# Jorgenlf/Drone-2d-custom-gym-env-for-reinforcement-learning

Measured on AMD Instinct MI355X. Metric: env-steps/sec at 65 536 parallel envs; 1/2/4/8 MI355X scaling, higher is better.
Workload: dtype f64

## Files before the change

### drone-2d-custom-gym-env-for-reinforcement-learning_amd/csrc/d2d_device.h

```cpp
#pragma once
#include <hip/hip_runtime.h>
#include <stdint.h>

#include "../../include/drone2d.h"
#include "d2d_pmath.h"

#pragma clang diagnostic ignored "-Wbitwise-instead-of-logical"

#ifdef D2D_BSTAMP
#define BST_N (1024 * 64 * 8)
__device__ uint64_t d2d_bst[BST_N];
#define BST_ARG , uint64_t* bst = nullptr
#define BST(k, dep)                                                                                      \
    do {                                                                                                 \
        if (bst) {                                                                                       \
            uint64_t bst_v;                                                                              \
            asm volatile("s_memtime %0\n\ts_waitcnt lgkmcnt(0)" : "=s"(bst_v) : "v"(dep));            \
            bst_t[k] = bst_v;                                                                            \
        }                                                                                                \
    } while (0)
#else
#define BST_ARG
#define BST(k, dep) \
    do {       \
// ... 564 lines not shown
        const double t = le ? xf : x;
        const int ti = le ? B.ixf : ix;
        const double tk = le ? B.kxf : kx;
        B.a = to_a ? t : a;
        B.b = to_a ? b : t;
        B.ia = to_a ? ti : B.ia;
        B.ka = to_a ? tk : B.ka;
        B.ib = to_a ? B.ib : ti;
        B.ixf = le ? ix : B.ixf;
        B.kxf = le ? kx : B.kxf;
        const int j = k + 1;
        const double nfulc = (le | c1) ? nfc : fulc;
        const int njf = (le | c1) ? jn : jf;
        const double nnfc = le ? xf : (c1 ? x : nfc);
        const int njn = le ? jx : (c1 ? j : jn);
        B.fulc = nfulc;
        B.nfc = nnfc;
        B.xf = le ? x : xf;
        jf = njf;
        jn = njn;
        jx = le ? j : jx;
    }
    T.snap[kind][k] = BtSnap{B.a, B.b, B.fulc, B.nfc, B.xf, B.rat, B.e, B.ka, B.kxf, B.num, B.ia, B.ib, B.ixf,
                             jf, jn, jx, 0};
    T.len[kind] = k;
}

__device__ __forceinline__ double bt_check(const BtIt& h, int k, double px, double py, double ffulc, double fnfc,
                                           double fx, int& dev) {
    const double fu = norm2(h.X - px, h.Y - py);
    const double r = h.dxn * (fx - ffulc);
    double q = h.dxf * (fx - fnfc);
    double p = h.dxf * q - h.dxn * r;
    q = 2.0 * (q - r);
    p = (q > 0.0) ? -p : p;
    q = fabs(q);
    const bool par = (fabs(p) < fabs(0.5 * q * h.e)) & (p > q * h.am) & (p < q * h.bm);
    const bool ok = !par & (fu <= fx);
    dev = min(dev, ok ? BT_HOT : k);
    return fu;
}

template <bool LT>
__device__ __forceinline__ BtIt bt_hot(const BtHot* hot, int kind, int j) {
    if (!LT) return hot->it[kind][j];
    using HL = __attribute__((address_space(3))) const double;
    const HL* q = (const HL*)&hot->it[kind][j];
    return BtIt{q[0], q[1], q[2], q[3], q[4], q[5], q[6], q[7]};
}
template <bool LT>
__device__ __forceinline__ double bt_dist(const BtHot* hot, int kind, int j, double px, double py) {
    const BtIt h = bt_hot<LT>(hot, kind, j);
    return norm2(h.X - px, h.Y - py);
}
struct BtLane {
    int kind, len, dev;
    double fa, fb, fc;
};
template <bool LT>
__device__ __forceinline__ BtLane bt_start(const BrTab& T, const BtHot* hot, double px, double py) {
    const double f0 = bt_dist<LT>(hot, 0, 0, px, py);
    const double f1 = bt_dist<LT>(hot, 0, 1, px, py);
    BtLane L;
    L.kind = (f1 <= f0) ? 1 : 0;
    L.len = T.len[L.kind];
    L.dev = L.len;
    L.fa = f0;
    L.fb = L.kind ? f0 : f1;
    L.fc = L.kind ? f1 : f0;
    return L;
}
template <bool LT>
__device__ __forceinline__ void bt_window(const BtHot* hot, BtLane& L, int k, double px, double py) {
    L.fa = bt_dist<LT>(hot, L.kind, k - 2, px, py);
    L.fb = bt_dist<LT>(hot, L.kind, k - 1, px, py);
    L.fc = bt_dist<LT>(hot, L.kind, k, px, py);
}
template <bool LT>
__device__ __forceinline__ void bt_verify(const BtHot* hot, BtLane& L, int k0, int k1, double px, double py) {
    double fa = L.fa, fb = L.fb, fc = L.fc;
    int dev = L.dev;
    const int kind = L.kind;
    for (int k = k0; __ballot(k < min(dev, k1)) != 0ull; k += 3) {
        BtIt ha{}, hb{}, hc{};
        if (LT || k < min(dev, k1)) {
            ha = bt_hot<LT>(hot, kind, k + 1);
            hb = bt_hot<LT>(hot, kind, k + 2);
            hc = bt_hot<LT>(hot, kind, k + 3);
        }
        const double fd = bt_check(ha, k, px, py, fa, fb, fc, dev);
        const double fe = bt_check(hb, k + 1, px, py, fb, fc, fd, dev);
        const double ff = bt_check(hc, k + 2, px, py, fc, fd, fe, dev);
        fa = fd;
        fb = fe;
        fc = ff;
    }
    L.dev = min(dev, L.len);
    L.fa = fa;
    L.fb = fb;
    L.fc = fc;
}
__device__ __forceinline__ void bt_restore(const BtSnap& S, Brent& B) {
    B.a = S.a;
    B.b = S.b;
    B.fulc = S.fulc;
    B.nfc = S.nfc;
    B.xf = S.xf;
    B.rat = S.rat;
    B.e = S.e;
    B.ka = S.ka;
    B.kxf = S.kxf;
    B.num = S.num;
    B.ia = S.ia;
    B.ib = S.ib;
    B.ixf = S.ixf;
}
template <bool LT>
__device__ __forceinline__ void bt_restore_f(const BtSnap& S, const BtHot* hot, int kind, double px, double py,
                                             Brent& B) {
    B.ffulc = bt_dist<LT>(hot, kind, S.j_fulc, px, py);
    B.fnfc = bt_dist<LT>(hot, kind, S.j_nfc, px, py);
    B.fx = bt_dist<LT>(hot, kind, S.j_xf, px, py);
}
template <bool LT, class SC>
__device__ __forceinline__ double bt_finish(const SC& s, const BrTab& T, const BtHot* hot, int kind, int dev,
                                            double px, double py, int& iu) {
    const BtSnap& S = T.snap[kind][dev];
    Brent B;
    bt_restore(S, B);
    if (__ballot(brent_active(B)) != 0ull) {
        const PathK K = path_k(s);
        bt_restore_f<LT>(S, hot, kind, px, py, B);
        brent_run(s, K, px, py, B);
    }
    iu = B.ixf;
    return B.xf;
}
template <bool LT, class S>
__device__ __forceinline__ double closest_u_tab(const S& s, const BrTab& T, const BtHot* hot, double px,
                                                double py, int& iu) {
    BtLane L = bt_start<LT>(T, hot, px, py);
    bt_verify<LT>(hot, L, 1, BT_K, px, py);
    return bt_finish<LT>(s, T, hot, L.kind, L.dev, px, py, iu);
}
__device__ __forceinline__ int bt_split(const BrTab& T) { return max(4, (T.len[0] + 3) / 2); }
#ifndef D2D_BT_EARLY
#define D2D_BT_EARLY 16
#endif
constexpr int BT_EARLY = D2D_BT_EARLY;
#ifndef D2D_BT_EARLY_GRP
#define D2D_BT_EARLY_GRP 0
#endif
static_assert(BT_EARLY == 0 || (BT_EARLY >= 4 && BT_EARLY % 3 == 1 && BT_EARLY < BT_K), "BT_EARLY");
__device__ __forceinline__ int bt_third(const BrTab& T, int p) {
    const int third = (T.len[0] + 2) / 3;
    return p == 0 ? 1 : (p >= 3 ? BT_K : 1 + p * third);
}
template <bool LT>
__device__ __forceinline__ void bt_window_snap(const BrTab& T, const BtHot* hot, BtLane& L, int k0, double px,
                                               double py) {
    const BtSnap& W = T.snap[L.kind][k0];
    L.fa = bt_dist<LT>(hot, L.kind, W.j_fulc, px, py);
    L.fb = bt_dist<LT>(hot, L.kind, W.j_nfc, px, py);
    L.fc = bt_dist<LT>(hot, L.kind, W.j_xf, px, py);
}

struct Body {
    double px, py, a, vx, vy, w;
};

constexpr double M_F = 0.2, M_M = 0.4;

__host__ __device__ constexpr double moment_box(double m, double w, double h) {
    double hw = w / 2.0, hh = h / 2.0;
    double vx[4] = {hw, hw, -hw, -hw}, vy[4] = {-hh, hh, hh, -hh};
    double s1 = 0.0, s2 = 0.0;
    for (int i = 0; i < 4; ++i) {
        double v1x = vx[i] + 0.0, v1y = vy[i] + 0.0;
        double v2x = vx[(i + 1) % 4] + 0.0, v2y = vy[(i + 1) % 4] + 0.0;
        double aa = v2x * v1y - v2y * v1x;
        double bb = (v1x * v1x + v1y * v1y) + (v1x * v2x + v1y * v2y) + (v2x * v2x + v2y * v2y);
        s1 += aa * bb;
        s2 += aa;
    }
    return (m * s1) / (6.0 * s2);
}
constexpr double MI_F = 1.0 / M_F, MI_M = 1.0 / M_M;
constexpr double II_F = 1.0 / moment_box(M_F, 100.0, 10.0);
constexpr double II_M = 1.0 / moment_box(M_M, 20.0, 20.0);

struct Arms {
    double m7c[2], m7s[2];
    double f47c, f47s, f40c, f40s, f33c, f33s;
};
__device__ __forceinline__ void arm(const Arms& A, int k, double& r1x, double& r1y, double& r2x, double& r2y) {
    const int m = k < 3 ? 0 : 1;
    const int q = k % 3;
    r1x = (q == 0) ? -A.m7c[m] : ((q == 1) ? 0.0 : A.m7c[m]);
    r1y = (q == 0) ? -A.m7s[m] : ((q == 1) ? 0.0 : A.m7s[m]);
    const double c = (k == 0 || k == 5) ? A.f47c : ((k == 1 || k == 4) ? A.f40c : A.f33c);
    const double s = (k == 0 || k == 5) ? A.f47s : ((k == 1 || k == 4) ? A.f40s : A.f33s);
    r2x = (k < 3) ? -c : c;
    r2y = (k < 3) ? -s : s;
}

constexpr int ARMS_N = 10;
__device__ __forceinline__ void arms_store(const Arms& A, double* ab, int stride) {
    const double v[ARMS_N] = {A.m7c[0], A.m7c[1], A.m7s[0], A.m7s[1], A.f47c, A.f47s,
                              A.f40c, A.f40s, A.f33c, A.f33s};
#pragma unroll
    for (int q = 0; q < 10; ++q) ab[q * stride] = v[q];
}
__device__ __forceinline__ void arm_lds(const double* ab, int stride, int k, double& r1x, double& r1y, double& r2x,
                                        double& r2y) {
    using LdsD = __attribute__((address_space(3))) double;
    const volatile LdsD* v = (const volatile LdsD*)ab;
    const int m = k < 3 ? 0 : 1;
    const int q = k % 3;
    const double mc = (q == 1) ? 0.0 : v[(0 + m) * stride], ms = (q == 1) ? 0.0 : v[(2 + m) * stride];
    r1x = (q == 0) ? -mc : ((q == 1) ? 0.0 : mc);
    r1y = (q == 0) ? -ms : ((q == 1) ? 0.0 : ms);
    const int f = (k == 0 || k == 5) ? 4 : ((k == 1 || k == 4) ? 6 : 8);
    const double c = v[f * stride], sn = v[(f + 1) * stride];
    r2x = (k < 3) ? -c : c;
    r2y = (k < 3) ? -sn : sn;
}

__device__ __forceinline__ void advance_position(Body& b) {
    b.px = fma(b.vx + 0.0, DT, b.px);
    b.py = fma(b.vy + 0.0, DT, b.py);
    b.a = fma(b.w + 0.0, DT, b.a);
}
template <class S>
__device__ __forceinline__ bool frame_hits(const S& s, const Body& F, double cs, double sn) {
    bool hit = false;
    for (int k = 0; k < s.n_circles; ++k) {
        const double dx = s.cx[k] - F.px, dy = s.cy[k] - F.py;
        {
            const double reach = s.cr[k] + 51.25;
            const bool near = (fabs(dx) < reach) & (fabs(dy) < reach);
            if (__ballot(near) == 0ull) continue;
        }
        const double lx = dx * cs + dy * sn;
        const double ly = -dx * sn + dy * cs;
        const double ex = lx - fmin(fmax(lx, -FRAME_HX), FRAME_HX), ey = ly - fmin(fmax(ly, -FRAME_HY), FRAME_HY);
        const double r = s.cr[k];
        hit |= (ex * ex + ey * ey <= r * r);
    }
    return hit;
}
template <class S>
__device__ __forceinline__ bool phys_positions(const S& s, Body B[3], double fL, double fR, double cs[3],
                                               double sn[3], double& fx, double& fy, double& tq) {
    double c0, s0;
    sincos_d(B[0].a, s0, c0);
    {
        const double tx = B[0].px - (0.0 * c0 - 0.0 * s0), ty = B[0].py - (0.0 * s0 + 0.0 * c0);
        const double cgx = c0 * 0.0 + (-s0) * 0.0 + tx, cgy = s0 * 0.0 + c0 * 0.0 + ty;
        double fwx = c0 * 0.0 + (-s0) * fL, fwy = s0 * 0.0 + c0 * fL;
        double rx = (c0 * -DRONE_R + (-s0) * 0.0 + tx) - cgx, ry = (s0 * -DRONE_R + c0 * 0.0 + ty) - cgy;
        fx = 0.0 + fwx;
        fy = 0.0 + fwy;
        tq = 0.0 + (rx * fwy - ry * fwx);
        fwx = c0 * 0.0 + (-s0) * fR;
        fwy = s0 * 0.0 + c0 * fR;
        rx = (c0 * DRONE_R + (-s0) * 0.0 + tx) - cgx;
        ry = (s0 * DRONE_R + c0 * 0.0 + ty) - cgy;
        fx = fx + fwx;
        fy = fy + fwy;
        tq += rx * fwy - ry * fwx;
    }
#pragma unroll
    for (int i = 0; i < 3; ++i) advance_position(B[i]);
    sincos_d(B[0].a, sn[0], cs[0]);
#pragma unroll
    for (int i = 1; i < 3; ++i) {
        const double d = B[i].a - B[0].a;
        if (!D2D_EXACT_TRIG && fabs(d) < 1e-2) {
            const double d2 = d * d;
            const double sd = d * fma(d2, fma(d2, fma(d2, -1.0 / 5040.0, 1.0 / 120.0), -1.0 / 6.0), 1.0);
            const double cdm1 = d2 * fma(d2, fma(d2, fma(d2, 1.0 / 40320.0, -1.0 / 720.0), 1.0 / 24.0), -0.5);
            sn[i] = fma(sn[0], cdm1, fma(cs[0], sd, sn[0]));
            cs[i] = fma(cs[0], cdm1, fma(-sn[0], sd, cs[0]));
        } else {
            sincos_d(B[i].a, sn[i], cs[i]);
        }
    }
    return frame_hits(s, B[0], cs[0], sn[0]);
}
template <class S>
__device__ __forceinline__ bool frame_advance(const S& s, Body& F) {
    advance_position(F);
    double sn, cs;
    sincos_d(F.a, sn, cs);
    return frame_hits(s, F, cs, sn);
}

__device__ __forceinline__ Arms make_arms(const double cs[3], const double sn[3]) {
    Arms A;
    A.m7c[0] = cs[1] * 7.0; A.m7s[0] = sn[1] * 7.0;
    A.m7c[1] = cs[2] * 7.0; A.m7s[1] = sn[2] * 7.0;
    A.f47c = cs[0] * 47.0; A.f47s = sn[0] * 47.0;
    A.f40c = cs[0] * 40.0; A.f40s = sn[0] * 40.0;
    A.f33c = cs[0] * 33.0; A.f33s = sn[0] * 33.0;
    return A;
}
// ... 385 lines not shown
```

### drone-2d-custom-gym-env-for-reinforcement-learning_amd/csrc/d2d_kernels.h

```cpp
#pragma once
#include <type_traits>

#include "d2d_curriculum.h"
#include "d2d_device.h"
#include "d2d_layout.h"

namespace d2dk {
using namespace d2d;

constexpr int BLOCK = 256;
constexpr int K1_THREADS = 256;
constexpr size_t K1_LDS_BUDGET = 40 * 1024;
constexpr size_t K2_LDS_BUDGET = 64 * 1024;
constexpr int PRIO_W0 = 2, PRIO_W1 = 1, PRIO_W2 = 3, PRIO_W3 = 1, PRIO_W2_POST = 0;

struct StepArgs {
    int n;
    int ns;
    int n_scn;
    double* st;
    int32_t* ist;
    double* acc;
    const void* scn;
    const BrTab* brt;
// ... 45 lines not shown
            a.stamps[(size_t)(blockIdx.x * (blockDim.x >> 6) + (threadIdx.x >> 6)) * 8 + 7] =                          \
                ((uint64_t)__builtin_amdgcn_s_getreg((3 << 11) | 20) << 32) |                          \
                (uint32_t)__builtin_amdgcn_s_getreg((31 << 11) | 4) | ((uint64_t)(wave & 3) << 36) |   \
                ((uint64_t)(uint32_t)(wg + 1) << 40);                                                  \
    } while (0)
#define D2D_FSTAMP_BASE 65536
#define FSTAMP(k)                                                                                      \
    do {                                                                                               \
        if (a.stamps && (threadIdx.x & 63) == 0)                                                       \
            a.stamps[D2D_FSTAMP_BASE + (size_t)(blockIdx.x * (blockDim.x >> 6) + (threadIdx.x >> 6)) * 8 + (k)] =      \
                __builtin_amdgcn_s_memtime();                                                          \
    } while (0)
#else
#define STAMP(k) \
    do {         \
    } while (0)
#define FSTAMP(k) \
    do {          \
    } while (0)
#endif

__device__ __forceinline__ const BrTab* brtab(const StepArgs& a, int si) { return a.brt ? a.brt + si : nullptr; }
__device__ __forceinline__ size_t rc_entry(const StepArgs& a, int i, uint32_t ep) {
    return (size_t)(ep & 1u) * (size_t)a.ns + (size_t)i;
}

template <bool LDS, int NT, class S>
__device__ __forceinline__ const S* stage_scenarios(const StepArgs& a, S* lds, int first = 0, int count = -1) {
    if (!LDS) return scn_tab<S>(a);
    if (count < 0) count = a.n_scn;
    const int words = count * (int)(sizeof(S) / 8);
    const double* src = reinterpret_cast<const double*>(scn_tab<S>(a) + first);
    double* dst = reinterpret_cast<double*>(lds);
    for (int k = threadIdx.x; k < words; k += NT) dst[k] = src[k];
    return lds - first;
}
template <int NT>
__device__ __forceinline__ const BtHot* stage_hot(const StepArgs& a, BtHot* lds, int first = 0, int count = -1) {
    if (count < 0) count = a.n_scn;
    const int per = (int)(sizeof(BtHot) / 16);
    for (int k = threadIdx.x; k < count * per; k += NT) {
        const double2* src = reinterpret_cast<const double2*>(&a.brt[first + k / per].hot) + (k % per);
        reinterpret_cast<double2*>(lds)[k] = *src;
    }
    return lds - first;
}
template <int NWAVES>
__device__ __forceinline__ void glds_copy(void* lds_dst, const void* gsrc, int bytes) {
    using LP = __attribute__((address_space(3))) void;
    using GP = __attribute__((address_space(1))) void;
    const int wave = __builtin_amdgcn_readfirstlane(threadIdx.x >> 6), lane = threadIdx.x & 63;
    for (int c = wave; c * 1024 < bytes; c += NWAVES) {
        const int off = c * 1024 + lane * 16;
        if (off < bytes)
            __builtin_amdgcn_global_load_lds((GP*)((const char*)gsrc + off), (LP*)((char*)lds_dst + c * 1024), 16, 0, 0);
    }
}

__device__ __forceinline__ size_t fidx(int f, int n, int i) { return (size_t)f * (size_t)n + (size_t)i; }
template <typename T>
__device__ __forceinline__ T& fld(T* base, int f, int n, int i) {
    T* fb = base + (size_t)__builtin_amdgcn_readfirstlane(f) * (size_t)__builtin_amdgcn_readfirstlane(n);
    return fb[i];
}

__device__ __forceinline__ Body load_frame(const StepArgs& a, int i) {
    const int n = a.ns;
    return Body{fld(a.st, 0, n, i), fld(a.st, 1, n, i), fld(a.st, 2, n, i),
                fld(a.st, 3, n, i), fld(a.st, 4, n, i), fld(a.st, 5, n, i)};
}
template <class SC>
__device__ __forceinline__ void spawn_state(const StepArgs& a, const SC& S, int i, uint32_t ep, double sp[7]) {
    double x, y, th;
    spawn_draw(S, a.seed, (uint32_t)a.cfg.env_id_base + (uint32_t)i, ep, x, y, th);
    double sl, cl, sr, cr;
    sincos_d(th + PI, sl, cl);
    sincos_d(th, sr, cr);
    sp[0] = x;
    sp[1] = y;
    sp[2] = th;
    sp[3] = cl * DRONE_R + x;
    sp[4] = sl * DRONE_R + y;
    sp[5] = cr * DRONE_R + x;
    sp[6] = sr * DRONE_R + y;
}

using LdsU32 = __attribute__((address_space(3))) uint32_t;
__device__ __forceinline__ bool flag_seen(const uint32_t& f) {
    return __builtin_amdgcn_readfirstlane(*(const volatile LdsU32*)&f) != 0u;
}
__device__ __forceinline__ int pool_scenario(const StepArgs& a, int j, uint32_t ep) {
    return *a.pool_base + (a.pool_n > 1 ? pool_pick(a.seed, (uint32_t)a.cfg.env_id_base + (uint32_t)j, ep, a.pool_n) : 0);
}
__device__ __forceinline__ int fresh_slot(int j, uint32_t ep) { return 2 * j + (int)(ep & 1u); }
enum { FR_HEAD = 0, FR_TAIL0 = 1, FR_TAIL1 = 2, FR_WORDS = 4 };
__device__ __forceinline__ int next_scenario(const StepArgs& a, int j, uint32_t ep) {
    if (a.cfg.scn_pool == 2) return fresh_slot(j, ep);
    if (a.cfg.scn_pool) return pool_scenario(a, j, ep);
    if (a.n_scn <= 1) return 0;
    return a.env_scn[j];
}

struct K1Shared {
    double cas[6][EPB];
    int scn[EPB];
    uint8_t cause[EPB];
    uint8_t cvalid[EPB];
    uint32_t pflags[EPB];
    uint32_t ep[EPB];
    double sina[EPB];
    uint32_t w0t[EPB], w0fl[EPB];
    uint32_t f_done, f_ca, f_gs, f_rp, f_ver, f_ver1, f_acc, n_tile;
    double pe[2][EPB];
    double acc[D2D_NSTATS][EPB];
    union {
        struct {
            double jb[6 * JB_PER_JOINT][EPB];
            double arms[ARMS_N][EPB];
        } g;
        struct {
            double post[7][EPB];
            alignas(16) float obs[EPB * D2D_OBS_DIM];
        } p;
    } u;
};

__device__ __forceinline__ int lane_fresh() {
    int l;
    asm volatile("v_mbcnt_lo_u32_b32 %0, -1, 0\n\tv_mbcnt_hi_u32_b32 %0, -1, %0" : "=v"(l));
    return l;
}
__device__ __forceinline__ void flag_raise(uint32_t& f) {
    __builtin_amdgcn_fence(__ATOMIC_RELEASE, "workgroup");
    if ((threadIdx.x & 63) == 0) *(volatile LdsU32*)&f = 1u;
}
__device__ __forceinline__ void flag_wait(const uint32_t& f) {
    while (!flag_seen(f)) __builtin_amdgcn_s_sleep(1)  ;
    __builtin_amdgcn_fence(__ATOMIC_ACQUIRE, "workgroup");
}
__device__ __forceinline__ void tile_arrive(uint32_t& c) {
    __builtin_amdgcn_fence(__ATOMIC_RELEASE, "workgroup");
    if ((threadIdx.x & 63) == 0) atomicAdd(&c, 1u);
}
__device__ __forceinline__ void tile_wait(const uint32_t& c, uint32_t n) {
    while (__builtin_amdgcn_readfirstlane(*(const volatile LdsU32*)&c) < n) __builtin_amdgcn_s_sleep(1);
    __builtin_amdgcn_fence(__ATOMIC_ACQUIRE, "workgroup");
}

template <bool LT, class SC>
__device__ __forceinline__ double bt_finish_join(const SC& s, const BrTab& T, const BtHot* hot, const BtLane& L,
                                                 const uint32_t& fv, const uint32_t& dv, double px, double py,
                                                 int& iu) {
    constexpr int IT_JOIN = 200;
    const PathK K = path_k(s);
    const bool early = L.dev < L.len;
    Brent B;
    bt_restore(T.snap[L.kind][L.dev], B);
    if (__ballot(early) != 0ull) {
        if (early) bt_restore_f<LT>(T.snap[L.kind][L.dev], hot, L.kind, px, py, B);
        uint32_t up = 0u;
        int it = 0;
        for (;; ++it) {
            if (!(early & brent_open(B) & (it < IT_JOIN) & (__builtin_amdgcn_readfirstlane(up) == 0u))) break;
            up = *(const volatile LdsU32*)&fv;
            brent_step(s, K, px, py, B);
        }
        B.num += it;
    }
    flag_wait(fv);
    const bool late = !early & ((dv < (uint32_t)L.len) | brent_active(B));
    if (__ballot(late) != 0ull) {
        if (late) {
            const BtSnap& S = T.snap[L.kind][min((uint32_t)L.len, dv)];
            bt_restore(S, B);
            bt_restore_f<LT>(S, hot, L.kind, px, py, B);
        }
    }
    if (__ballot(brent_active(B)) != 0ull) brent_run(s, K, px, py, B, nullptr, 500 - (BT_K_MAX + 1) - IT_JOIN);
    iu = B.ixf;
    return B.xf;
}

template <bool LDS, bool LTAB, bool GRP, class S>
__device__ __forceinline__ void k1_stage(const StepArgs& a, S* s_scn, int wg, const S*& scns,
                                         const BtHot*& hots, int& s0) {
    const int ws = (GRP && LDS) ? a.wg_scn[wg] : 0;
    s0 = ws >= 0 ? ws : -ws - 2;
    const int ncopy = (GRP && LDS) ? (ws >= 0 ? 1 : 2) : a.n_scn;
    hots = nullptr;
    if (LDS && (ncopy == 1 || !LTAB)) {
        glds_copy<K1_THREADS / 64>(s_scn, scn_tab<S>(a) + s0, (int)sizeof(S) * ncopy);
        if (LTAB) glds_copy<K1_THREADS / 64>(s_scn + 1, &a.brt[s0].hot, (int)sizeof(BtHot));
        scns = s_scn - s0;
        if (LTAB) hots = reinterpret_cast<const BtHot*>(s_scn + 1) - s0;
    } else {
        scns = stage_scenarios<LDS, K1_THREADS>(a, s_scn, s0, ncopy);
        if (LTAB) hots = stage_hot<K1_THREADS>(a, reinterpret_cast<BtHot*>(s_scn + ncopy), s0, ncopy);
    }
}

extern __shared__ __attribute__((aligned(16))) uint4 d2d_dyn_lds[];
constexpr int K1_KN_BYTES = D2D_MAX_WPS * 64 * 8;
template <bool LDS, bool LTAB, bool GRP, bool S3, class SC>
__device__ __forceinline__ void k1_body(const StepArgs& a, const SC* scns, const BtHot* hots, int s0, K1Shared& sh,
                                        int wg, int role, int qt) {
    const int wave = role;
    const int lane = threadIdx.x & 63;
    const bool gvalid = wg >= 0;
    const int e0 = gvalid ? wg * EPB : 0;
    const int i = e0 + lane;
    const int ie = (GRP && gvalid) ? a.lane_env[i] : i;
    const bool valid = gvalid && (GRP ? ie >= 0 : i < a.n);
    const int n = a.ns;
    const bool auto_reset = a.cfg.auto_reset != 0;
    constexpr bool EARLY = LDS && LTAB && !S3 && BT_EARLY > 0 && (!GRP || D2D_BT_EARLY_GRP);
    STAMP(0);
    if (wg == 0 && qt == 0 && a.fill_ctl)
        __hip_atomic_store(&a.fill_ctl[0], __hip_atomic_load(&a.fill_ctl[1], __ATOMIC_RELAXED, __HIP_MEMORY_SCOPE_AGENT),
                           __ATOMIC_RELAXED, __HIP_MEMORY_SCOPE_AGENT);
    if (wg == 0 && qt == 0 && a.clock)
        __hip_atomic_fetch_add(a.clock, (int64_t)1, __ATOMIC_RELAXED, __HIP_MEMORY_SCOPE_AGENT);
    if (wave == 0) sh.scn[lane] = (valid && a.env_scn && a.n_scn > 1) ? a.env_scn[ie] : s0;
    if (S3 && wave == 0) sh.pflags[lane] = 0x7fffffffu;
    Body PF{};
    if (valid && wave != 0) PF = load_frame(a, i);
    if (qt == 0) {
        sh.f_done = 0u;
        sh.f_ca = 0u;
        sh.f_gs = 0u;
        sh.f_rp = 0u;
        sh.f_ver = 0u;
        sh.f_ver1 = 0u;
        sh.f_acc = 0u;
        sh.n_tile = 0u;
    }
    __syncthreads();
    STAMP(1);
    const SC& S = scns[sh.scn[lane]];
    float* const trow = a.tobs ? a.tobs + (size_t)ie * D2D_OBS_DIM : nullptr;
    float* const orow = &sh.u.p.obs[lane * D2D_OBS_DIM];

    Body F0{};
    double path_err = 0.0, tot_rew = 0.0;
    int t = 0, cause = 0;
    uint32_t flags = 0;
    RewardVel RV{};
    double dclose = 0.0, rew_sum = 0.0, rew_pp = 0.0, pdist = 0.0;
    uint32_t plal = 0;
    bool done = false;
    if (wave == 0) {
        __builtin_amdgcn_s_setprio(PRIO_W0);
        double ov[19];
        Body B[3];
        double j[12], cs[3], sn[3], fx = 0.0, fy = 0.0, tq = 0.0;
        if (valid) {
#pragma unroll
            for (int b = 0; b < 3; ++b) {
                B[b].px = fld(a.st, 6 * b + 0, n, i);
                B[b].py = fld(a.st, 6 * b + 1, n, i);
                B[b].a = fld(a.st, 6 * b + 2, n, i);
                B[b].vx = fld(a.st, 6 * b + 3, n, i);
                B[b].vy = fld(a.st, 6 * b + 4, n, i);
                B[b].w = fld(a.st, 6 * b + 5, n, i);
            }
#pragma unroll
            for (int k = 0; k < 12; ++k) j[k] = fld(a.st, D2D_S_J + k, n, i);
            t = fld(a.ist, D2D_I_T, n, i);
            flags = (uint32_t)fld(a.ist, D2D_I_FLAGS, n, i);
            const float2 act = reinterpret_cast<const float2*>(a.act)[ie];
            const float fs = (float)a.cfg.force_scale;
            const float lf = __fmul_rn(__fadd_rn(act.x / 2.0f, 0.5f), fs);
            const float rf = __fmul_rn(__fadd_rn(act.y / 2.0f, 0.5f), fs);
            if (phys_positions(S, B, (double)lf, (double)rf, cs, sn, fx, fy, tq)) flags |= D2D_FLAG_COLLIDED;
            t += 1;
            cause = end_cause(a.cfg, S, B[0], (flags & D2D_FLAG_COLLIDED) != 0, t);
            done = cause != 0;
            const int32_t ep = fld(a.ist, D2D_I_EPISODE, n, i);
            const bool cv = done && auto_reset && a.rc_tag[rc_entry(a, i, (uint32_t)ep)] == ep;
            sh.ep[lane] = (uint32_t)ep;
            sh.cause[lane] = (uint8_t)cause;
            sh.sina[lane] = sn[0];
            sh.cvalid[lane] = cv ? 1u : 0u;
            sh.w0t[lane] = (uint32_t)t;
            sh.w0fl[lane] = flags;
            if (!(done && auto_reset)) {
#pragma unroll
                for (int b = 0; b < 3; ++b) {
                    fld(a.st, 6 * b + 0, n, i) = B[b].px;
                    fld(a.st, 6 * b + 1, n, i) = B[b].py;
                    fld(a.st, 6 * b + 2, n, i) = B[b].a;
                }
            }
        }
        flag_raise(sh.f_done);
        if (valid) {
            const Arms A = make_arms(cs, sn);
            const double pos[6] = {B[0].px, B[0].py, B[1].px, B[1].py, B[2].px, B[2].py};
            double vel[9] = {B[0].vx, B[0].vy, B[0].w, B[1].vx, B[1].vy, B[1].w, B[2].vx, B[2].vy, B[2].w};
            phys_velocities<true>(A, pos, a.damping_dt, fx, fy, tq, vel, j, &sh.u.g.jb[0][lane], EPB,
                                  &sh.u.g.arms[0][lane]);
            asm volatile("" ::: "memory");
            const int ln = lane_fresh(), iw = e0 + ln;
            const uint32_t cw = sh.cause[ln];
            cause = (int)cw;
            done = cw != 0u;
            t = (int)sh.w0t[ln];
            flags = sh.w0fl[ln];
            if (!(done && auto_reset)) {
// ... 76 lines not shown
            __builtin_amdgcn_s_setprio(PRIO_W2);
            if (valid && a.brt) {
                const BrTab& T = a.brt[sh.scn[lane]];
                const BtHot* hot = LTAB ? hots + sh.scn[lane] : &T.hot;
                Body F = PF;
                advance_position(F);
                BtLane L = bt_start<LTAB>(T, hot, F.px, F.py);
                const int k0 = bt_third(T, 1), k1 = bt_third(T, 2);
                if (k0 < min(k1, L.len)) {
                    if (k0 >= 4) bt_window<LTAB>(hot, L, k0, F.px, F.py);
                else bt_window_snap<LTAB>(T, hot, L, k0, F.px, F.py);
                    bt_verify<LTAB>(hot, L, k0, k1, F.px, F.py);
                }
                atomicMin(&sh.pflags[lane], (uint32_t)L.dev);
            }
            flag_raise(sh.f_ver1);
        }
        __builtin_amdgcn_s_setprio(PRIO_W1);
        if (valid) {
            Body F = PF;
            advance_position(F);
            double so[19];
            sensor_pos(a.cfg, S, F.px, F.py, F.a, so);
            const CAStatic C = ca_static(a.cfg, S, so);
            sh.cas[0][lane] = C.d;
            sh.cas[1][lane] = C.os;
            sh.cas[2][lane] = C.oc;
            sh.cas[3][lane] = C.lpa;
            sh.cas[4][lane] = C.lca;
            sh.cas[5][lane] = C.rr;
#pragma unroll
            for (int k = 0; k < 19; ++k) row[k] = (float)so[k];
        }
        flag_raise(sh.f_ca);
        flag_wait(sh.f_done);
        if (valid) {
            done = sh.cause[lane] != 0u;
            need = done && auto_reset;
            if (done && trow) {
#pragma unroll
                for (int k = 3; k < 17; ++k) trow[k] = row[k];
            }
        }
        if (__ballot(need) != 0ull) {
            if (need) {
                if (sh.cvalid[lane] != 0u) {
                    const float* c = a.rc_obs + rc_entry(a, i, sh.ep[lane]) * D2D_OBS_DIM;
#pragma unroll
                    for (int k = 0; k < 19; ++k) row[k] = c[k];
                } else {
                    const uint32_t ep = sh.ep[lane];
                    const SC& SN = scns[next_scenario(a, ie, ep)];
                    double sp[7], so[19];
                    spawn_state(a, SN, ie, ep, sp);
                    sensor_obs(a.cfg, SN, Body{sp[0], sp[1], sp[2], 0.0, 0.0, 0.0}, so);
#pragma unroll
                    for (int k = 0; k < 19; ++k) row[k] = (float)so[k];
                }
            }
        }
        STAMP(4);
        flag_wait(sh.f_gs);
        STAMP(5);
        if (valid) {
            if (need) {
#pragma unroll
                for (int k = 0; k < 19; ++k) orow[k] = row[k];
            } else {
#pragma unroll
                for (int k = 3; k < 17; ++k) orow[k] = row[k];
            }
        }
        tile_arrive(sh.n_tile);
    } else if (wave == 2) {
        __builtin_amdgcn_s_setprio(PRIO_W2);
        double po[8];
        Body F{};
        if (valid) {
            F = PF;
            advance_position(F);
            uint32_t f = (uint32_t)fld(a.ist, D2D_I_FLAGS, n, i);
            const BrTab* T = brtab(a, sh.scn[lane]);
            if (T) {
                const BtHot* hot = LTAB ? hots + sh.scn[lane] : &T->hot;
                BtLane L = bt_start<LTAB>(*T, hot, F.px, F.py);
                int iu;
                double u;
                if constexpr (EARLY) {
                    bt_verify<LTAB>(hot, L, 1, BT_EARLY, F.px, F.py);
                    u = bt_finish_join<LTAB>(S, *T, hot, L, sh.f_ver, sh.pflags[lane], F.px, F.py, iu);
                } else {
                    bt_verify<LTAB>(hot, L, 1, !LDS ? BT_K : S3 ? bt_third(*T, 1) : bt_split(*T), F.px, F.py);
                    flag_wait(sh.f_ver);
                    if (S3) flag_wait(sh.f_ver1);
                    L.dev = min(L.dev, (int)sh.pflags[lane]);
                    u = bt_finish<LTAB>(S, *T, hot, L.kind, L.dev, F.px, F.py, iu);
                }
                path_obs_u(a.cfg, S, F.px, F.py, F.a, u, f, po, iu);
            } else {
                path_obs<LTAB, SC::RM>(a.cfg, S, T, F.px, F.py, F.a, f, po, LTAB ? hots + sh.scn[lane] : nullptr,
                                       SC::RM ? reinterpret_cast<double*>(d2d_dyn_lds) : nullptr);
            }
            sh.pflags[lane] = f & D2D_FLAG_LA_LOCK;
        }
        STAMP(4);
        __builtin_amdgcn_s_setprio(PRIO_W2_POST);
        flag_wait(sh.f_done);
        flag_wait(sh.f_ca);
        RewardPos RP{};
        RewardPath RQ{};
        bool d = false;
        if (valid) {
            const int cause = (int)sh.cause[lane];
            d = cause != 0;
            CAStatic C;
            C.lpa = sh.cas[3][lane];
            RP = reward_pos(a.cfg, F, cause, sh.sina[lane]);
            RQ = reward_path(a.cfg, RP, C, po);
        }
        flag_wait(sh.f_gs);
        if (valid) {
            if (!(d && auto_reset)) {
#pragma unroll
                for (int k = 0; k < 8; ++k) orow[19 + k] = (float)po[k];
            }
            if (d && trow) {
#pragma unroll
                for (int k = 0; k < 8; ++k) trow[19 + k] = (float)po[k];
            }
        }
        if (valid) {
            sh.u.p.post[0][lane] = RQ.ls;
            sh.u.p.post[1][lane] = RQ.lc;
            sh.u.p.post[2][lane] = RQ.pa;
            sh.u.p.post[3][lane] = RQ.dist;
            sh.u.p.post[4][lane] = RP.aa;
            sh.u.p.post[5][lane] = RP.coll;
            sh.u.p.post[6][lane] = RP.reach;
        }
        flag_raise(sh.f_rp);
        tile_arrive(sh.n_tile);
        STAMP(5);
    } else {
        __builtin_amdgcn_s_setprio(PRIO_W2);
        double po[8];
        if (!LDS) {
            sh.pflags[lane] = 0x7fffffffu;
        } else if (valid && a.brt) {
            const BrTab& T = a.brt[sh.scn[lane]];
            const BtHot* hot = LTAB ? hots + sh.scn[lane] : &T.hot;
            Body F = PF;
            advance_position(F);
            BtLane L = bt_start<LTAB>(T, hot, F.px, F.py);
            const int k0 = EARLY ? BT_EARLY : S3 ? bt_third(T, 2) : bt_split(T);
            if (k0 < L.len) {
                if (k0 >= 4) bt_window<LTAB>(hot, L, k0, F.px, F.py);
                else bt_window_snap<LTAB>(T, hot, L, k0, F.px, F.py);
                bt_verify<LTAB>(hot, L, k0, BT_K, F.px, F.py);
            }
            if (S3) atomicMin(&sh.pflags[lane], (uint32_t)L.dev);
            else sh.pflags[lane] = (uint32_t)L.dev;
        }
        flag_raise(sh.f_ver);
        __builtin_amdgcn_s_setprio(PRIO_W3);
        if (valid) {
            sh.pe[0][lane] = fld(a.st, D2D_S_PATH_ERR, n, i);
            sh.pe[1][lane] = fld(a.st, D2D_S_TOT_REW, n, i);
        }
        flag_wait(sh.f_done);
        const bool cv = valid && sh.cvalid[lane] != 0u;
        if (valid) done = sh.cause[lane] != 0u;
        if (valid && done) {
#pragma unroll
            for (int k = 0; k < D2D_NSTATS; ++k) sh.acc[k][lane] = fld(a.acc, k, n, i);
        }
        flag_raise(sh.f_acc);
        if (valid && done && auto_reset) {
            const uint32_t ep = sh.ep[lane];
            const int nscn = next_scenario(a, ie, ep);
            const SC& SN = scns[nscn];
            double sp[7];
            spawn_state(a, SN, ie, ep, sp);
            uint32_t rfl = 0;
            if (cv) {
                const size_t ce = rc_entry(a, i, ep);
                const float* c = a.rc_obs + ce * D2D_OBS_DIM + 19;
#pragma unroll
                for (int k = 0; k < 8; ++k) po[k] = (double)c[k];
                rfl = (uint32_t)a.rc_rfl[ce];
            } else {
                path_obs(a.cfg, SN, brtab(a, nscn), sp[0], sp[1], sp[2], rfl, po);
            }
            const double th = sp[2];
            const double bodies[18] = {sp[0], sp[1], th, 0.0, 0.0, 0.0, sp[3], sp[4], th, 0.0, 0.0, 0.0,
                                       sp[5], sp[6], th, 0.0, 0.0, 0.0};
#pragma unroll
            for (int f = 0; f < 18; ++f) fld(a.st, f, n, i) = bodies[f];
#pragma unroll
            for (int k = 0; k < 12; ++k) fld(a.st, D2D_S_J + k, n, i) = 0.0;
            fld(a.st, D2D_S_PATH_ERR, n, i) = 0.0;
            fld(a.st, D2D_S_TOT_REW, n, i) = 0.0;
            fld(a.ist, D2D_I_T, n, i) = 0;
            fld(a.ist, D2D_I_FLAGS, n, i) = (int32_t)rfl;
            fld(a.ist, D2D_I_EPISODE, n, i) = (int32_t)(ep + 1u);
            if (a.cfg.scn_pool && a.env_scn) a.env_scn[ie] = nscn;
        }
        if (!LDS && a.fq) {
            const bool need = valid && done && auto_reset;
            const uint64_t m = __ballot(need);
            if (m != 0ull) {
                const int first = __ffsll((unsigned long long)m) - 1;
                uint32_t base = 0;
                if (lane == first) base = atomicAdd(&a.fqc[FR_HEAD], (uint32_t)__popcll(m));
                base = __shfl(base, first);
                const uint32_t pos = base + (uint32_t)__popcll(m & ((1ull << lane) - 1ull));
                if (need) a.fq[pos & a.fq_mask] = fresh_slot(ie, sh.ep[lane] + 1u);
            }
        }
        STAMP(4);
        flag_wait(sh.f_gs);
        STAMP(5);
        if (valid && done && auto_reset) {
#pragma unroll
            for (int k = 0; k < 8; ++k) orow[19 + k] = (float)po[k];
        }
        tile_arrive(sh.n_tile);
    }
    STAMP(2);

    if (wave != 0) {
        tile_wait(sh.n_tile, 4u);
        STAMP(3);
        constexpr int TT = K1_THREADS - 64;
        const int tq = qt - 64;
        if (GRP) {
            for (int k = tq; gvalid && k < EPB * D2D_OBS_DIM; k += TT) {
                const int r = k / D2D_OBS_DIM;
                const int e = a.lane_env[e0 + r];
                if (e >= 0) a.obs[(size_t)e * D2D_OBS_DIM + (k - r * D2D_OBS_DIM)] = sh.u.p.obs[k];
            }
        } else {
            const int rows = gvalid ? max(0, min(EPB, a.n - e0)) : 0;
            const int words = rows * D2D_OBS_DIM;
            float* dst = a.obs + (size_t)e0 * D2D_OBS_DIM;
            int k0 = 0;
            if (rows == EPB && ((uintptr_t)a.obs & 15u) == 0) {
                float4* d4 = reinterpret_cast<float4*>(dst);
                const float4* s4 = reinterpret_cast<const float4*>(sh.u.p.obs);
                for (int k = tq; k < words / 4; k += TT) d4[k] = s4[k];
                k0 = words;
            }
            for (int k = k0 + tq; k < words; k += TT) dst[k] = sh.u.p.obs[k];
        }
    } else {
        if (S3) flag_wait(sh.f_acc);
        STAMP(3);
    }
    const int lne = lane_fresh(), ile = e0 + lne, iee = GRP ? ie : ile;
    const bool vle = gvalid && (GRP ? iee >= 0 : ile < a.n);
    if (wave == 0 && vle) {
        const int lane = lne, i = ile, ie = iee;
        if (S3) {
            path_err = sh.pe[0][lane];
            tot_rew = sh.pe[1][lane];
        }
        flags = (flags & ~D2D_FLAG_LA_LOCK) | (GRP ? sh.pflags[lane] : plal);
        const double reward = rew_sum;
        path_err += GRP ? sh.u.p.post[3][lane] : pdist;
        const double ape_g = GRP ? path_err / (double)t : 0.0;
        tot_rew += reward;
        bool trunc = false, term = done;
        if (a.cfg.timeup_truncates && done && cause == D2D_END_TIMEUP) {
            trunc = true;
            term = false;
        }
        const int io = ie;
        a.rew[io] = (float)reward;
        a.term[io] = (uint8_t)term;
        a.trunc[io] = (uint8_t)trunc;
        if (a.info) {
            float* r = a.info + (size_t)ie * D2D_INFO_DIM;
            r[D2D_INFO_CA] = (float)RV.cal;
            r[D2D_INFO_PA] = (float)sh.u.p.post[2][lane];
            r[D2D_INFO_PP] = (float)rew_pp;
            r[D2D_INFO_COLL] = (float)sh.u.p.post[5][lane];
            r[D2D_INFO_REACH] = (float)sh.u.p.post[6][lane];
            r[D2D_INFO_AA] = (float)sh.u.p.post[4][lane];
            r[D2D_INFO_DCLOSE] = (float)dclose;
            r[D2D_INFO_STEPS] = (float)t;
            r[D2D_INFO_CAUSE] = (float)cause;
            r[D2D_INFO_APE] = done ? (float)(GRP ? ape_g : path_err / (double)t) : 0.0f;
            r[D2D_INFO_TOTREW] = done ? (float)tot_rew : 0.0f;
            r[D2D_INFO_REWARD] = (float)reward;
        }
        if (done) {
            double pacc[D2D_NSTATS];
#pragma unroll
            for (int k = 0; k < D2D_NSTATS; ++k) pacc[k] = sh.acc[k][lane];
            const double ape = GRP ? ape_g : path_err / (double)t;
            const bool c1 = cause & D2D_END_COLLISION, c2 = cause & D2D_END_REACH;
            const bool c4 = cause & D2D_END_TIMEUP, c5 = cause & D2D_END_AA;
            fld(a.acc, D2D_ST_RETURN, n, i) = pacc[D2D_ST_RETURN] + tot_rew;
            fld(a.acc, D2D_ST_EPISODES, n, i) = pacc[D2D_ST_EPISODES] + 1.0;
            fld(a.acc, D2D_ST_SUCCESS, n, i) = pacc[D2D_ST_SUCCESS] + (c2 ? 1.0 : 0.0);
            fld(a.acc, D2D_ST_FAIL, n, i) = pacc[D2D_ST_FAIL] + ((c1 || c4 || c5) ? 1.0 : 0.0);
            fld(a.acc, D2D_ST_COLLISION, n, i) = pacc[D2D_ST_COLLISION] + ((c1 && !c2 && !c4 && !c5) ? 1.0 : 0.0);
            fld(a.acc, D2D_ST_APE, n, i) = pacc[D2D_ST_APE] + ape;
// ... 373 lines not shown
```

Baseline: 2.534 billion.

## Let undecided lanes ride Brent steps from early snapshot while verifier runs

Adds a 'rider' mode: lanes not yet proven to diverge early start Brent iteration from the BT_EARLY snapshot during the wait for the verifier, instead of idling. After the flag arrives, riders whose state bit-matches the tabulated snapshot jump to the verifier's divergence point; otherwise they continue. The verifier window start moves by BT_RIDE so it checks only beyond the riders' coverage. This overlaps otherwise idle wave time with useful work, at the cost of extra restore and compare logic and more divergent control flow.

New measurement: 2.565 billion, median of 6. 1.2% higher.

```diff
diff --git a/drone-2d-custom-gym-env-for-reinforcement-learning_amd/csrc/d2d_device.h b/drone-2d-custom-gym-env-for-reinforcement-learning_amd/csrc/d2d_device.h
--- a/drone-2d-custom-gym-env-for-reinforcement-learning_amd/csrc/d2d_device.h
+++ b/drone-2d-custom-gym-env-for-reinforcement-learning_amd/csrc/d2d_device.h
@@ -740,6 +740,11 @@
 #define D2D_BT_EARLY_GRP 0
 #endif
 static_assert(BT_EARLY == 0 || (BT_EARLY >= 4 && BT_EARLY % 3 == 1 && BT_EARLY < BT_K), "BT_EARLY");
+#ifndef D2D_BT_RIDE
+#define D2D_BT_RIDE 15
+#endif
+constexpr int BT_RIDE = D2D_BT_RIDE;
+static_assert(BT_RIDE >= 0 && (BT_RIDE == 0 || BT_EARLY > 0) && BT_EARLY + BT_RIDE < BT_K, "BT_RIDE");
 __device__ __forceinline__ int bt_third(const BrTab& T, int p) {
     const int third = (T.len[0] + 2) / 3;
     return p == 0 ? 1 : (p >= 3 ? BT_K : 1 + p * third);
diff --git a/drone-2d-custom-gym-env-for-reinforcement-learning_amd/csrc/d2d_kernels.h b/drone-2d-custom-gym-env-for-reinforcement-learning_amd/csrc/d2d_kernels.h
--- a/drone-2d-custom-gym-env-for-reinforcement-learning_amd/csrc/d2d_kernels.h
+++ b/drone-2d-custom-gym-env-for-reinforcement-learning_amd/csrc/d2d_kernels.h
@@ -221,8 +221,59 @@
                                                  const uint32_t& fv, const uint32_t& dv, double px, double py,
                                                  int& iu) {
     constexpr int IT_JOIN = 200;
+    static_assert(BT_RIDE < IT_JOIN, "the riders' passes end below the first loop's cap");
     const PathK K = path_k(s);
     const bool early = L.dev < L.len;
+    if constexpr (BT_RIDE > 0) {
+        const bool rider = !early & (L.len > BT_EARLY);
+        const bool any_rider = __ballot(rider) != 0ull;
+        Brent B;
+        bt_restore(T.snap[L.kind][rider ? BT_EARLY : L.dev], B);
+        if (__ballot(early) != 0ull) {
+            if (early) bt_restore_f<LT>(T.snap[L.kind][L.dev], hot, L.kind, px, py, B);
+        }
+        if (rider) {
+            B.ffulc = L.fa;
+            B.fnfc = L.fb;
+            B.fx = L.fc;
+        }
+        const bool in = early | rider;
+        uint32_t up = 0u;
+        int it = 0;
+        for (;; ++it) {
+            const bool open = in & brent_open(B);
+            const bool go = (any_rider & (it < BT_RIDE)) |
+                            ((__builtin_amdgcn_readfirstlane(up) == 0u) & (__ballot(early & open) != 0ull));
+            if (!(open & (it < IT_JOIN) & go)) break;
+            up = *(const volatile LdsU32*)&fv;
+            brent_step(s, K, px, py, B);
+        }
+        B.num += it;
+        flag_wait(fv);
+        const uint32_t m = min((uint32_t)L.len, dv);
+        bool jump = false;
+        if (__ballot(rider & brent_open(B)) != 0ull) {
+            const int q = min(BT_EARLY + it, L.len);
+            const BtSnap& Q = T.snap[L.kind][q];
+            const auto same = [](double x, double y) { return __double_as_longlong(x) == __double_as_longlong(y); };
+            const bool eq = same(B.a, Q.a) & same(B.b, Q.b) & same(B.fulc, Q.fulc) & same(B.nfc, Q.nfc) &
+                            same(B.xf, Q.xf) & same(B.rat, Q.rat) & same(B.e, Q.e) & (B.ia == Q.ia) &
+                            (B.ib == Q.ib) & (B.ixf == Q.ixf);
+            jump = rider & brent_open(B) & (it >= BT_RIDE) & eq & (m >= (uint32_t)q);
+        }
+        const bool late = jump | (!in & ((dv < (uint32_t)L.len) | brent_active(B)));
+        if (__ballot(late) != 0ull) {
+            if (late) {
+                const BtSnap& S = T.snap[L.kind][m];
+                bt_restore(S, B);
+                if (brent_active(B)) bt_restore_f<LT>(S, hot, L.kind, px, py, B);
+            }
+        }
+        if (__ballot(brent_active(B)) != 0ull)
+            brent_run(s, K, px, py, B, nullptr, 500 - (BT_K_MAX + 1) - IT_JOIN);
+        iu = B.ixf;
+        return B.xf;
+    }
     Brent B;
     bt_restore(T.snap[L.kind][L.dev], B);
     if (__ballot(early) != 0ull) {
@@ -605,7 +656,7 @@
             Body F = PF;
             advance_position(F);
             BtLane L = bt_start<LTAB>(T, hot, F.px, F.py);
-            const int k0 = EARLY ? BT_EARLY : S3 ? bt_third(T, 2) : bt_split(T);
+            const int k0 = EARLY ? BT_EARLY + BT_RIDE : S3 ? bt_third(T, 2) : bt_split(T);
             if (k0 < L.len) {
                 if (k0 >= 4) bt_window<LTAB>(hot, L, k0, F.px, F.py);
                 else bt_window_snap<LTAB>(T, hot, L, k0, F.px, F.py);
```
